# line/open-universe

Measured on AMD Instinct MI355X. Metric: real_time_factor (audio s / wall s), UNIVERSE++ 16 kHz 8-step enhance, higher is better.
Workload: dtype f32; 1 GPU; UNIVERSE++ 16 kHz, 8 diffusion steps, batch=1 utterance(s) of 4 s per GPU per step; network=PP16, n_diffusion_steps=8, batch_per_gpu=1, samples_per_utterance=64000, launches_per_enhance=414

## Files before the change

### open-universe_amd/csrc/ou_api.cpp

```cpp
#include <hip/hip_runtime.h>

#include <cmath>
#include <cstdio>
#include <cstdlib>
#include <cstring>
#include <map>
#include <string>
#include <vector>

#include "../../include/ouniverse.h"
#include "../../include/ouniverse_tuning.h"
#include "ou_kernels.h"
#include "ou_model.h"

using namespace ou;

namespace {
thread_local std::string g_last_error;
constexpr int kMaxSteps = 256;
constexpr size_t kProfSlots = 32768;
constexpr float kInvSqrt2 = 0.70710678118654752440f;
constexpr size_t align256(size_t bytes) { return (bytes + 255) & ~size_t(255); }

struct TensorRef {
  size_t off;
  int C, T;
};
struct Options {
  int dbg = 0, xcd_map = -1, conv_direct = 5, fuse = -1, fuse_nc = 0, rate_small = 1, fuse_upfir = 1, block3 = 0, d4_fir = 1,
      d4_force = 0, d4_short = 1, d2_wk = 0, wino = 1, d2_map = -1, unfuse64 = 0, preact = 1;
  int gru_v = 2, gru_bmax = 0, gru_ts = 0, gru_upw = 0, gru_backoff = 0, gru_agent = -1, gru_dbg = 0;
  int split = -1;
  int dbg_dec0_under_gru = 0;
  int tile_prefetch = 1;
  int trace = 0, no_overlap = 0, ts = 0, deep_factor = 8, mask_fused = 1, split_wino = 1, d2_tile_rule = 1;
  int ens_share = 1;
  double tile_min = -1.0;
  std::string chain_ts;
};
}

struct ou_packer {
  Model m;
  std::map<std::string, HostTensor> sd;
  std::vector<float> blob;
  std::string err;
};

struct ou_handle {
  Model m;
  const float* W = nullptr;
  int device = 0;
  int num_cu = 256;
  std::string err;
  std::map<std::string, TensorRef> tensors;
  int n_launch = 0, n_conv = 0;
  int cond_B = 0, cond_T = 0;
  bool trace = false;
  Options opt;
  std::string plan_with_options;
  int last_cfg = -1;
  long long* tstamps = nullptr;
  std::map<size_t, float> alphas;
  hipStream_t aux[3] = {nullptr, nullptr, nullptr};
  std::vector<hipEvent_t> events;
  size_t ev_used = 0;
  bool overlap = true;
  int force_cfg = -1, force_sc = 0;
  bool profile = false;
  struct ProfRec { double flops, bytes; int cfg; };
  std::vector<ProfRec> prof;
  size_t prof_used = 0;
  unsigned long long* prof_dev = nullptr;
  int fuse_mode = -1;
  int fuse_nc = 0;
  struct WsRec { const void* ws; size_t bytes; int B, T; };
  std::vector<WsRec> ws_ready;
  int gru_agent_stores = 0;
  int lanes = 1, lane = 0;
  int lane_max_b = 0;
  struct NoiseSource {
    bool on = false;
    unsigned long long seed = 0;
    std::vector<unsigned long long> streams;
    float* scratch = nullptr;
    size_t scratch_bytes = 0;
  } noise_src;
  double plane_per_sample = 0.0, wav_plane_per_sample = 0.0;
  bool ws_ok(const void* ws, size_t bytes, int B, int T) const {
    (void)T;
    for (const WsRec& r : ws_ready)
      if (r.ws == ws) return r.B == B && r.bytes <= bytes;
    return false;
  }
};

namespace {

int fail(ou_handle* h, int code, const std::string& msg) {
  if (h) h->err = msg;
  g_last_error = msg;
  return code;
}

struct Tensor {
  float* p = nullptr;
  int C = 0, T = 0;
};

struct OptDesc {
  const char* key;
  int Options::*ip;
  double Options::*dp;
  bool experiments_only;
  const char* doc;
};
const OptDesc kOptions[] = {
    {"conv_direct", &Options::conv_direct, nullptr, false, "kernel generations the conv launcher may use (0 .. 5, ConvArgs::direct)"},
    {"split", &Options::split, nullptr, false, "-1 rule / 0 never / 1 wherever possible: conv_split_kernel (bf16-split operands)"},
    {"split_wino", &Options::split_wino, nullptr, false, "experiments build: 0 = the plain bf16-split kernel also where its minimal-filtering form would take the layer"},
    {"wino", &Options::wino, nullptr, false, "0: never the minimal-filtering (Winograd / Cook-Toom) kernel variants"},
    {"fuse", &Options::fuse, nullptr, false, "-1 cost model / 0 never / 2 / 3: depth of the fused ConvBlock body (conv_chain kernels)"},
    {"fuse_nc", &Options::fuse_nc, nullptr, false, "128 / 256: columns per tile of the fused ConvBlock body (0: launcher's choice)"},
    {"fuse_upfir", &Options::fuse_upfir, nullptr, false, "0: up-path anti-alias FIR always as its own pass"},
    {"rate_small", &Options::rate_small, nullptr, false, "0: outermost rate-change convs on the generic kernels (no rate_down / rate_up)"},
    {"preact", &Options::preact, nullptr, false, "0: every PReLU in its consumer's operand path (ConvArgs::out_act never set)"},
    {"unfuse64", &Options::unfuse64, nullptr, false, "1: 64-channel ConvBlock bodies as three split-K launches"},
    {"block3", &Options::block3, nullptr, false, "1: the three body convs of a deep-level ConvBlock in one launch (experiments build only)"},
    {"xcd_map", &Options::xcd_map, nullptr, false, "block -> tile mapping of the LDS-tiled conv kernel (-1: launcher's choice)"},
    {"d2_map", &Options::d2_map, nullptr, false, "block -> tile mapping of the wide-load split-K kernels (-1: launcher's choice)"},
    {"d2_tile_rule", &Options::d2_tile_rule, nullptr, false, "0: round 5's 64- vs 32-column rule of the wide-load split-K kernels (ignores that only 64-column tiles have minimal filtering)"},
    {"d2_wk", &Options::d2_wk, nullptr, false, "4 / 8: K slices of conv_direct2_kernel (0: launcher's rule)"},
    {"d4_fir", &Options::d4_fir, nullptr, false, "0: up convs with a fusable FIR stay on the first-generation fused kernel"},
    {"d4_short", &Options::d4_short, nullptr, false, "0: the 401-frame levels at batch 1 stay on the first-generation kernels"},
    {"d4_force", &Options::d4_force, nullptr, false, "10 TM + log2(WK): that conv_direct4 tile shape wherever a layer admits it"},
    {"tile_min", nullptr, &Options::tile_min, false, "wave tiles per SIMD from which the no-split-K kernels take a layer (< 0: 1.2)"},
    {"tile_prefetch", &Options::tile_prefetch, nullptr, false, "0: no LDS prefetch of the epilogue operand in conv_direct3_kernel"},
    {"deep_factor", &Options::deep_factor, nullptr, false, "blocks of 64 x 128 per CU up to which a layer counts as 'deep' (split-K kernels)"},
    {"mask_fused", &Options::mask_fused, nullptr, false, "ragged batches: 0 = a separate tail-mask launch after EVERY producer (reference form of the masks)"},
    {"gru_v", &Options::gru_v, nullptr, false, "2 ring kernel / 1 polling-wave kernel (experiments build)"},
    {"gru_bmax", &Options::gru_bmax, nullptr, false, "cap on the utterances per GRU launch (forces the chunked path)"},
    {"gru_upw", &Options::gru_upw, nullptr, false, "hidden units per workgroup of the ring kernel (0: from the batch size)"},
    {"gru_backoff", &Options::gru_backoff, nullptr, false, "poll back-off experiments of the ring kernel (0: none)"},
    {"gru_agent_stores", &Options::gru_agent, nullptr, false, "-1 handle's mode / 0 plain / 1 agent-scope publishes"},
    {"gru_dbg", &Options::gru_dbg, nullptr, false, "bit 0 no republish safety net, bit 1 system-scope publishes, bit 2 FAULT INJECTION (tests)"},
    {"gru_ts", &Options::gru_ts, nullptr, false, "1: per-wave cycle stamps of the GRU kernel into the end of the workspace (tuning)"},
    {"ts", &Options::ts, nullptr, false, "1: per-wave phase stamps in ou_bench_conv (tuning)"},
    {"trace", &Options::trace, nullptr, false, "1: one line per conv launch on stderr"},
    {"no_overlap", &Options::no_overlap, nullptr, false, "1: no side streams inside a call (every kernel alone on the device)"},
    {"ens_share", &Options::ens_share, nullptr, false, "ou_enhance_ensemble: 1 = conditioner once over the B inputs, its results replicated; 0 = over all E * B rows"},
    {"dbg", &Options::dbg, nullptr, true, "phase ablation switches of the conv kernels: WRONG results by design"},
    {"dbg_dec0", &Options::dbg_dec0_under_gru, nullptr, true, "first decoder block under the GRU: upper-bound measurement, WRONG results"},
};
constexpr int kNumOptions = (int)(sizeof(kOptions) / sizeof(kOptions[0]));
const OptDesc* find_option(const char* key) {
  for (int i = 0; i < kNumOptions; i++)
    if (std::strcmp(kOptions[i].key, key) == 0) return &kOptions[i];
  return nullptr;
}
using EnvCfg = Options;

struct Runner {
  ou_handle* h;
  EnvCfg env;
  char* base;
  size_t cap;
  size_t off = 0;
  bool dry;
  hipStream_t st;
  int B;
  hipError_t herr = hipSuccess;
  bool oom = false;
  const char* where = "";
  size_t max_plane = 0;
  bool mel_scale_preset = false;

  Runner(ou_handle* h_, void* ws, size_t cap_, bool dry_, hipStream_t st_, int B_)
      : h(h_), env(h_->opt), base((char*)ws), cap(cap_), dry(dry_), st(st_), B(B_), main_st(st_) {
#ifndef OU_EXPERIMENTS
    env.dbg = 0; env.dbg_dec0_under_gru = 0;
#endif
  }

  float* alloc_raw(size_t floats) {
    size_t bytes = align256(floats * 4);
    size_t o = off;
// ... 67 lines not shown
    const float* res = nullptr;
    float res_scale = 1.f;
    const float* in_scale = nullptr;
    bool act = true;
    const float* fir = nullptr;
    int fir_len = 0;
    const float* fir_bias = nullptr;
    bool rate_down = false;
    bool rate_up = false;
    bool out_act = false;
    float out_alpha = 1.f;
    bool no_mask = false;
  };
  bool stored_act = false;
  bool unsupported = false;
  std::vector<ConvArgs>* collect = nullptr;
  unsigned* status_words = nullptr;
  unsigned long long* block3_bar = nullptr;
  int gru_area_rows = 0;
  bool gru_shared = false;
  hipEvent_t pre_gru = nullptr;
  bool want_pre_gru = false;
  static int gru_share_of(int lanes, int B, bool overlap) {
    const int ncl = 2 * B < 8 ? 2 * B : 8;
    const int by_lanes = lanes > 1 ? (ncl * lanes + 7) / 8 : 1;
    return by_lanes * (overlap ? 2 : 1);
  }

  Tensor conv(const ConvL& L, const Tensor& in, const std::string& name, const Epi& e, const Tensor* dst = nullptr) {
    int Nq, Tout;
    if (L.stride > 1) { Nq = in.T / L.stride; Tout = Nq; }
    else { Nq = in.T; Tout = in.T * L.up; }
    Tensor out = dst ? *dst : alloc(name, L.Cout, Tout);
    if (dry || !ok()) return out;
    ConvArgs a;
    a.x = in.p; a.w = W(L.w_off); a.bias = W(L.b_off); a.y = out.p;
    if (L.KWP) { a.wd = W(L.wd_off); a.wu = W(L.wu_off); }
    if (L.ws_on) a.wsplit = W(L.ws_off);
    if (L.wsw_on) a.wsplitw = W(L.wsw_off);
    a.split = env.split; a.split_wino = env.split_wino;
    a.in_scale = e.in_scale;
    a.act = (L.act && e.act) ? 1 : 0;
    a.alpha_val = a.act ? h->alphas[L.a_off] : 0.f;
    a.add = e.add; a.add_scale = e.add_scale;
    a.film = e.film; a.film_bstride = e.film_bstride;
    a.res = e.res; a.res_scale = e.res_scale;
    if (e.out_act && !collect && !e.fir && !e.rate_down && !e.rate_up) { a.out_act = 1; a.out_alpha = e.out_alpha; }
    stored_act = false;
    if (e.fir && !e.rate_down) { a.fir = e.fir; a.fir_len = e.fir_len; a.bias = e.fir_bias; }
    if (e.rate_down) { a.fir = e.fir; a.fir_len = e.fir ? e.fir_len : 0; }
    a.B = B; a.Cin = L.Cin; a.Tin = in.T; a.Cout = L.Cout; a.M = L.M; a.Mp = L.Mp; a.KW = L.KW;
    a.stride = L.stride; a.pad = L.pad; a.up = L.up; a.CK = L.CK; a.Nq = Nq; a.Tout = Tout;
    a.force_cfg = h->force_cfg; a.force_sc = h->force_sc;
    a.dbg = env.dbg; a.force_xcd_map = env.xcd_map; a.direct = env.conv_direct; a.d4_fir_unfused = env.d4_fir; a.d4_force = env.d4_force; a.d4_short = env.d4_short; a.deep_factor = env.deep_factor; a.d2_tile_rule = env.d2_tile_rule; a.d2_wk = env.d2_wk; a.wino = env.wino; a.d2_map = env.d2_map;
    a.tile_min = env.tile_min; a.tile_prefetch = env.tile_prefetch;
    a.tstamps = h->tstamps;
    if (ragged && env.mask_fused && !e.no_mask) a.lens = lens_of(Tout);
    if (collect) { collect->push_back(a); return out; }
    int cfg = -1;
    if (h->profile && h->prof_dev && h->prof_used < kProfSlots) {
      ou_handle::ProfRec rec;
      const int kref = L.KW;
      rec.flops = 2.0 * L.M * (double)Nq * L.Cin * kref * B;
      rec.bytes = 4.0 * ((double)B * ((double)L.Cin * in.T + (double)L.Cout * Tout) + (double)L.M * L.Cin * kref);
      rec.cfg = -1;
      a.prof = h->prof_dev + 32 * h->prof_used;
      h->prof.push_back(rec);
      h->prof_used++;
    }
    unsupported = false;
    if (e.rate_down) {
      chk(launch_rate_down(a, st, &cfg), L.name.c_str());
    } else if (e.rate_up) {
      chk(launch_rate_up(a, st, &cfg), L.name.c_str());
    } else {
      hipError_t le = launch_conv(a, h->num_cu, st, &cfg);
      if (le == hipErrorNotSupported && a.out_act) {
        a.out_act = 0;
        le = launch_conv(a, h->num_cu, st, &cfg);
      }
      stored_act = a.out_act != 0;
      if (le == hipErrorNotSupported && e.fir) {
        if (a.prof) { h->prof.pop_back(); h->prof_used--; }
        unsupported = true;
        return out;
      }
      chk(le, L.name.c_str());
    }
    if (a.prof) h->prof.back().cfg = cfg;
    h->last_cfg = cfg;
    if (!e.no_mask && !(a.lens && conv_masks_rows(cfg))) mask(out);
    if (h->trace)
      std::fprintf(stderr, "OU_TRACE conv %-64s cfg=%d M=%d Nq=%d K=%d(Cin=%d KW=%d CK=%d) stride=%d up=%d B=%d MFLOP=%.1f\n",
                   name.c_str(), cfg, L.M, Nq, L.Cin * L.KW, L.Cin, L.KW, L.CK, L.stride, L.up, B,
                   2.0 * L.M * Nq * L.Cin * L.KW * B * 1e-6);
    h->n_conv++;
    return out;
  }

  struct BlockOut { Tensor h_next, v, c1; };
  int plan_chain(const BlockL& Bk, int T) {
    h->fuse_mode = env.fuse; h->fuse_nc = env.fuse_nc;
    if (h->fuse_mode == 0) return 0;
    if (ragged && !env.mask_fused) return 0;
    if (h->fuse_mode < 0 && Bk.C % 16 == 0 && Bk.c1.KWP && Bk.c2.KWP && Bk.c3.KWP) {
      if (env.conv_direct >= 3 && direct3_tiles_per_simd(Bk.C, T, B, h->num_cu) >= 1.9 && T >= 1024) return 0;
      if (env.unfuse64 && env.conv_direct >= 5 && env.wino && Bk.C % 64 == 0 && T >= 1024) return 0;
// ... 2335 lines not shown
```

### open-universe_amd/csrc/ou_conv_direct4.hip

```cpp
#include "ou_kernels.h"
#include "ou_internal.h"
#include "ou_dev.h"

#include <cmath>
#include <cstdlib>
#include <type_traits>

namespace ou {

typedef float f32x4acc __attribute__((ext_vector_type(4)));

template <int R, int TM, int WN, int WK, int D>
__global__ __launch_bounds__(64 * WN * WK) void conv_direct4_kernel(ConvArgs p) {
  constexpr int TN = 4, LPS = 2 * R, BM = 16 * TM, NW = WN * WK, EP = 68;
  static_assert(WN == 1 || WK == 1, "a block is either WN column tiles or WK slices of the reduction");
  static_assert(TM >= 1 && TM <= 4, "16 .. 64-row tiles");
  static_assert(D * LPS <= 60, "loads in flight must fit vmcnt");
  static_assert(D == 2 || D == 4, "ring depth");
  typedef float f32x3 __attribute__((ext_vector_type(3)));
  typedef typename std::conditional<TM == 4, f32x4, typename std::conditional<TM == 3, f32x3,
          typename std::conditional<TM == 2, f32x2, float>::type>::type>::type avec;
  extern __shared__ __attribute__((aligned(16))) float smem[];
  const int tid = threadIdx.x, lane = tid & 63;
  const int wv = __builtin_amdgcn_readfirstlane(tid >> 6);
  const int wn = WK == 1 ? wv : 0, wk = WK == 1 ? 0 : wv;
  const int L = blockIdx.x, q8 = L >> 3;
  int rg, cidx;
  if (p.xcd_map == 1) {
    const int gm8 = (p.grid_m + 7) >> 3;
    rg = (q8 % gm8) * 8 + (L & 7);
    cidx = q8 / gm8;
  } else {
    rg = q8 % p.grid_m;
    cidx = (q8 / p.grid_m) * 8 + (L & 7);
  }
  const int b = cidx / p.grid_n, chunk = cidx - b * p.grid_n;
  const int n0 = (chunk * WN + wn) * 64, m0 = rg * BM;
  if (b >= p.B || rg >= p.grid_m) return;
  if (WK == 1 && n0 >= p.Nq) return;
  if (p.prof && tid == 0) atomicMin(p.prof + (blockIdx.x & 15), (unsigned long long)__builtin_amdgcn_s_memrealtime());
  const int l15 = lane & 15, kk = lane >> 4;
  const int Tin = p.Tin, Mp = p.Mp, CK = p.CK, lck = 31 - __clz(CK);
  const float alpha = p.act ? p.alpha_val : 1.0f;
  const u32x4 rx = direct_desc(p.x + (size_t)b * p.Cin * Tin, (unsigned)p.Cin * (unsigned)Tin * 4u);
  const u32x4 rw = direct_desc(p.w, (unsigned)p.Cin * (unsigned)R * (unsigned)Mp * 4u);
  const int avo = (kk * Mp + m0 + TM * l15) * 4;
  const int c0 = n0 + TN * l15;
  const int bvo = c0 < p.Nq ? (kk * Tin + c0 * R) * 4 : (int)0x80000000;

  const int NS = (p.Cin >> 2) / WK;
  avec a4[D][R];
  f32x4 b4[D][R];
#pragma unroll
  for (int d0 = 0; d0 < D; d0++)
#pragma unroll
    for (int k = 0; k < R; k++) {
      if constexpr (TM == 4) a4[d0][k] = f32x4{0.f, 0.f, 0.f, 0.f};
      else if constexpr (TM == 3) a4[d0][k] = f32x3{0.f, 0.f, 0.f};
      else if constexpr (TM == 2) a4[d0][k] = f32x2{0.f, 0.f};
      else a4[d0][k] = 0.f;
      b4[d0][k] = f32x4{0.f, 0.f, 0.f, 0.f};
    }
  f32x4acc acc[TM][TN];
#pragma unroll
  for (int i = 0; i < TM; i++)
#pragma unroll
    for (int j = 0; j < TN; j++) acc[i][j] = f32x4acc{0.f, 0.f, 0.f, 0.f};

#define OU_ISSUE(g_, d)                                                                                                  \
  {                                                                                                                      \
    const int c4 = (wk + WK * (g_)) * 4;                                                                                 \
    const int wrow = ((c4 >> lck) * R) * CK + (c4 & (CK - 1));                   \
    const int xso = c4 * Tin * 4;                                                                                        \
    _Pragma("unroll") for (int k = 0; k < R; k++) {                                                                      \
      if constexpr (TM == 4)                                                                                             \
        asm volatile("buffer_load_dwordx4 %0, %1, %2, %3 offen" : "+v"(a4[d][k]) : "v"(avo), "s"(rw), "s"((wrow + k * CK) * Mp * 4)); \
      else if constexpr (TM == 3)                                                                                        \
        asm volatile("buffer_load_dwordx3 %0, %1, %2, %3 offen" : "+v"(a4[d][k]) : "v"(avo), "s"(rw), "s"((wrow + k * CK) * Mp * 4)); \
      else if constexpr (TM == 2)                                                                                        \
        asm volatile("buffer_load_dwordx2 %0, %1, %2, %3 offen" : "+v"(a4[d][k]) : "v"(avo), "s"(rw), "s"((wrow + k * CK) * Mp * 4)); \
      else                                                                                                               \
        asm volatile("buffer_load_dword %0, %1, %2, %3 offen" : "+v"(a4[d][k]) : "v"(avo), "s"(rw), "s"((wrow + k * CK) * Mp * 4)); \
    }                                                                                                                    \
    _Pragma("unroll") for (int k = 0; k < R; k++)                                                                        \
      asm volatile("buffer_load_dwordx4 %0, %1, %2, %3 offen offset:%4" : "+v"(b4[d][k]) : "v"(bvo), "s"(rx), "s"(xso), "n"(16 * k)); \
  }
#define OU_MMA(d, out)                                                                                                   \
  {                                                                                                                      \
    asm volatile("s_waitcnt vmcnt(%0)" ::"n"((out) * LPS));                                                              \
    _Pragma("unroll") for (int k = 0; k < R; k++) { asm volatile("" : "+v"(a4[d][k])); asm volatile("" : "+v"(b4[d][k])); } \
    float X[4 * R];                                                                                                      \
    _Pragma("unroll") for (int k = 0; k < R; k++) {                                                                      \
// ... 6 lines not shown
        if constexpr (TM == 1) av = a4[d][k]; else av = a4[d][k][i];                                                     \
        _Pragma("unroll") for (int j = 0; j < TN; j++)                                                                   \
          acc[i][j] = __builtin_amdgcn_mfma_f32_16x16x4f32(av, X[j * R + k], acc[i][j], 0, 0, 0);                        \
      }                                                                                                                  \
  }
  const bool ts_on = p.tstamps != nullptr;
  long long tc0 = 0, tc1 = 0, tc2 = 0, tr0 = 0;
  if (ts_on) { tr0 = (long long)__builtin_amdgcn_s_memrealtime(); tc0 = __builtin_readcyclecounter(); }
  if constexpr (D == 4) {
    OU_ISSUE(0, 0); OU_ISSUE(1, 1); OU_ISSUE(2, 2); OU_ISSUE(3, 3);
    if (ts_on) tc1 = __builtin_readcyclecounter();
    const int NR = NS / 4;
    for (int r = 0; r + 1 < NR; r++) {
      const int g = r * 4;
      OU_MMA(0, 3); OU_ISSUE(g + 4, 0);
      OU_MMA(1, 3); OU_ISSUE(g + 5, 1);
      OU_MMA(2, 3); OU_ISSUE(g + 6, 2);
      OU_MMA(3, 3); OU_ISSUE(g + 7, 3);
    }
    OU_MMA(0, 3); OU_MMA(1, 2); OU_MMA(2, 1); OU_MMA(3, 0);
  } else {
    OU_ISSUE(0, 0); OU_ISSUE(1, 1);
    if (ts_on) tc1 = __builtin_readcyclecounter();
    const int NR = NS / 2;
    for (int r = 0; r + 1 < NR; r++) {
      const int g = r * 2;
      OU_MMA(0, 1); OU_ISSUE(g + 2, 0);
      OU_MMA(1, 1); OU_ISSUE(g + 3, 1);
    }
    OU_MMA(0, 1); OU_MMA(1, 0);
  }
  if (ts_on) tc2 = __builtin_readcyclecounter();
#undef OU_ISSUE
#undef OU_MMA

  float* Ew = smem + (size_t)wv * BM * EP;
#pragma unroll
  for (int i = 0; i < TM; i++)
#pragma unroll
    for (int r = 0; r < 4; r++)
      *reinterpret_cast<f32x4*>(&Ew[(TM * (4 * kk + r) + i) * EP + 4 * l15]) =
          f32x4{acc[i][0][r], acc[i][1][r], acc[i][2][r], acc[i][3][r]};
  if constexpr (WK > 1) asm volatile("s_waitcnt lgkmcnt(0)\n\ts_barrier" ::: "memory");
  else asm volatile("s_waitcnt lgkmcnt(0)" ::: "memory");

  const int rt = WK == 1 ? lane : tid;
  constexpr int RNT = WK == 1 ? 64 : 64 * WK;
  const float* Er = WK == 1 ? Ew : smem;
  const float* filmb = p.film ? p.film + (size_t)b * p.film_bstride : nullptr;
  const size_t ybase = (size_t)b * p.Cout * p.Tout;
  const float insc = p.in_scale ? p.in_scale[b] : 1.0f;
  const int nvalid = p.Nq - n0;
  const int rlen = ragged_len(p.lens, b);
  if (p.up == 1) {
    constexpr int NQ = BM * 16, QPT = (NQ + RNT - 1) / RNT;
#pragma unroll
    for (int u = 0; u < QPT; u++) {
      const int e = rt + u * RNT;
      if (NQ % RNT != 0 && e >= NQ) break;
      const int row = e >> 4, cq = (e & 15) * 4;
      const int m = m0 + row;
      if (m >= p.M || cq >= nvalid) continue;
      const size_t idx = ybase + (size_t)m * p.Tout + n0 + cq;
      const bool full = cq + 4 <= nvalid;
      f32x4 ad = {0.f, 0.f, 0.f, 0.f}, rs = {0.f, 0.f, 0.f, 0.f};
      if (full) {
        if (p.add) ad = *reinterpret_cast<const f32x4u*>(p.add + idx);
        if (p.res) rs = *reinterpret_cast<const f32x4u*>(p.res + idx);
      } else {
#pragma unroll
        for (int s = 0; s < 4; s++) {
          if (p.add && cq + s < nvalid) ad[s] = p.add[idx + s];
          if (p.res && cq + s < nvalid) rs[s] = p.res[idx + s];
        }
      }
      f32x4 v = *reinterpret_cast<const f32x4*>(&Er[row * EP + cq]);
#pragma unroll
      for (int k = 1; k < WK; k++) v += *reinterpret_cast<const f32x4*>(&Er[(k * BM + row) * EP + cq]);
      if (p.in_scale) v *= insc;
      v += p.bias[m];
      if (p.add) v = (v + ad) * p.add_scale;
      if (filmb) v = filmb[m] * v + filmb[p.Cout + m];
      if (p.res) v = (v + rs) * p.res_scale;
      if (p.lens) v = ragged_mask4(v, n0 + cq, rlen);
      if (full) {
        *reinterpret_cast<f32x4u*>(p.y + idx) = v;
      } else {
#pragma unroll
        for (int s = 0; s < 4; s++)
          if (cq + s < nvalid) p.y[idx + s] = v[s];
      }
    }
  } else {
    const int up = p.up;
    const int m_hi = (m0 + BM - 1 < p.M - 1) ? m0 + BM - 1 : p.M - 1;
    const int co_lo = (int)__umulhi((unsigned)m0, p.magic_up);
    const int nco = (int)__umulhi((unsigned)m_hi, p.magic_up) - co_lo + 1;
    const int qpc = 16 * up;
    const int total = nco * qpc;
    for (int e = rt; e < total; e += RNT) {
      const int cl = (int)__umulhi((unsigned)(e >> 4), p.magic_up);
      const int tl = (e - cl * qpc) * 4;
      const int co = co_lo + cl;
      const int q0 = (int)__umulhi((unsigned)tl, p.magic_up);
      int ph = tl - q0 * up, q = q0;
      f32x4 v;
      bool ok[4];
// ... 244 lines not shown
    o[0] = tr0; o[1] = tc1 - tc0; o[2] = tc2 - tc1; o[3] = tc3 - tc2; o[4] = tc4 - tc3; o[5] = tc5 - tc4; o[6] = twait;
    o[7] = (long long)__builtin_amdgcn_s_memrealtime();
  }
  if (p.prof && tid == 0) atomicMin(p.prof + 16 + (blockIdx.x & 15), ~(unsigned long long)__builtin_amdgcn_s_memrealtime());
}

struct Direct4wCfg {
  int KW, TM, WK;
  void (*kern)(ConvArgs);
};
#define OU_D4W(KW, TM, WK) {KW, TM, WK, conv_direct4w_kernel<KW, TM, WK>}
static const Direct4wCfg kDirect4wCfgs[] = {OU_D4W(3, 1, 8), OU_D4W(3, 2, 8), OU_D4W(5, 1, 8), OU_D4W(5, 2, 8),
                                            OU_D4W(3, 1, 4), OU_D4W(3, 2, 4), OU_D4W(5, 1, 4), OU_D4W(5, 2, 4)};
hipError_t launch_conv_direct4w(const ConvArgs& a, int num_cu, hipStream_t stream, int* cfg_out) {
  if (!a.wu || a.stride != 1 || a.up != 1 || (a.KW != 3 && a.KW != 5) || a.pad != (a.KW - 1) / 2 || a.fir || a.Cin % 16 ||
      (a.in_scale != nullptr && a.act))
    return hipErrorInvalidConfiguration;
  if ((long)a.Cin * a.Tin * 4 >= (1L << 31) || (long)a.Cin * a.Mp * 8 * 4 >= (1L << 31)) return hipErrorInvalidConfiguration;
  const bool forced = a.force_cfg >= 600 && a.force_cfg < 800;
  if (!forced && !(a.wino && a.direct >= 5)) return hipErrorInvalidConfiguration;
  const int slots = a.Cin / 4;
  const long ct = (a.Nq + 63) / 64;
  int tm = 0, wk = 8;
  if (forced) {
    tm = ((a.force_cfg % 100) / 10);
    wk = a.force_cfg >= 700 ? 4 : 8;
  } else {
    const long b64 = (long)((a.M + 31) / 32) * ct * a.B;
    if (a.Nq >= 1024 || b64 * 10 >= (long)num_cu * 8) return hipErrorInvalidConfiguration;
    long best = 0;
    for (int t = 1; t <= 2; t++) {
      const long blocks = (long)((a.M + 16 * t - 1) / (16 * t)) * ct * a.B;
      const long cost = (blocks + num_cu - 1) / num_cu * t;
      if (!tm || cost <= best) { tm = t; best = cost; }
    }
  }
  if (tm < 1 || tm > 2 || slots % (wk * 4) != 0) return hipErrorInvalidConfiguration;
  const Direct4wCfg* c = nullptr;
  for (const Direct4wCfg& k : kDirect4wCfgs)
    if (k.KW == a.KW && k.TM == tm && k.WK == wk) { c = &k; break; }
  if (!c) return hipErrorInvalidConfiguration;
  ConvArgs aa = a;
  const long gy = (a.M + 16 * tm - 1) / (16 * tm);
  aa.grid_m = (int)gy;
  aa.grid_n = (int)ct;
  const long nblocks = 8L * ((gy + 7) / 8) * ct * a.B;
  if (cfg_out) *cfg_out = (wk == 4 ? 700 : 600) + 10 * tm + a.KW;
  hipLaunchKernelGGL(c->kern, dim3((unsigned)nblocks), dim3(64 * wk), (size_t)wk * 16 * tm * 68 * 4, stream, aa);
  return hipGetLastError();
}

struct Direct4Cfg {
  int R, TM, WN, WK, D;
  void (*kern)(ConvArgs);
};
#define OU_D4(R, TM, WN, WK, D) {R, TM, WN, WK, D, conv_direct4_kernel<R, TM, WN, WK, D>}
#ifdef OU_EXPERIMENTS
#define OU_D4_SHAPES(R, D)                                                                                    \
  OU_D4(R, 4, 4, 1, D), OU_D4(R, 2, 4, 1, D), OU_D4(R, 4, 1, 2, D), OU_D4(R, 2, 1, 2, D), OU_D4(R, 4, 1, 4, D), \
  OU_D4(R, 2, 1, 4, D), OU_D4(R, 4, 1, 8, D), OU_D4(R, 2, 1, 8, D), OU_D4(R, 1, 1, 4, D), OU_D4(R, 1, 1, 8, D), \
  OU_D4(R, 3, 1, 4, D), OU_D4(R, 3, 1, 8, D)
#else
#define OU_D4_SHAPES(R, D)                                                                            \
  OU_D4(R, 2, 4, 1, D), OU_D4(R, 2, 1, 2, D), OU_D4(R, 2, 1, 4, D), OU_D4(R, 2, 1, 8, D), OU_D4(R, 1, 1, 4, D), \
  OU_D4(R, 1, 1, 8, D), OU_D4(R, 3, 1, 4, D), OU_D4(R, 3, 1, 8, D)
#endif
static const Direct4Cfg kDirect4Cfgs[] = {
    OU_D4_SHAPES(1, 4), OU_D4_SHAPES(2, 4), OU_D4_SHAPES(3, 2), OU_D4_SHAPES(4, 2), OU_D4_SHAPES(5, 2), OU_D4_SHAPES(8, 2),
};
static size_t direct4_smem(const Direct4Cfg& c) { return (size_t)c.WN * c.WK * 16 * c.TM * 68 * 4; }
hipError_t init_direct4_kernels() {
  for (const Direct4Cfg& c : kDirect4Cfgs) {
    if (direct4_smem(c) <= 64 * 1024) continue;
    hipError_t e = hipFuncSetAttribute(reinterpret_cast<const void*>(c.kern), hipFuncAttributeMaxDynamicSharedMemorySize,
                                       (int)direct4_smem(c));
    if (e != hipSuccess) return e;
  }
  return hipSuccess;
}

static bool direct4_pick(int M, long ct_b, int slots, int R, int D, bool short_layer, int num_cu, int* tm_out, int* wk_out) {
  if (short_layer) {
    int wk = 8;
    while (wk > 4 && slots % (wk * D) != 0) wk >>= 1;
    if (slots % (wk * D)) return false;
    int best_tm = 0;
    long best_cost = 0;
    for (int tm = 1; tm <= 3; tm++) {
      const long blocks = (long)((M + 16 * tm - 1) / (16 * tm)) * ct_b;
      const long cost = (blocks + num_cu - 1) / num_cu * tm;
      if (!best_tm || cost <= best_cost) { best_tm = tm; best_cost = cost; }
    }
    *tm_out = best_tm; *wk_out = wk;
    return true;
  }
  const long tiles = (long)((M + 31) / 32) * ct_b;
  int wk = 8;
  while (wk > 1 && (slots % (wk * D) != 0 || (slots / wk) * 8 * R < 64 || tiles * wk > 12000)) wk >>= 1;
  if (slots % (wk * D)) return false;
  *tm_out = 2; *wk_out = wk;
  return true;
}

hipError_t launch_conv_direct4(const ConvArgs& a, int num_cu, hipStream_t stream, int* cfg_out, bool probe) {
  const int R = a.stride > 1 ? a.stride : 1;
  if (a.KW != R || a.pad != 0 || (a.stride > 1 && (a.up != 1 || a.Tin != a.Nq * R)) || a.Cin % 16 || a.CK % 4 || a.fir ||
      (a.in_scale != nullptr && a.act))
    return hipErrorInvalidConfiguration;
  if ((long)a.Cin * a.Tin * 4 >= (1L << 31) || (long)a.Cin * a.KW * a.Mp * 4 >= (1L << 31)) return hipErrorInvalidConfiguration;
  if (a.up > 1 && (a.Cout * a.up != a.M || a.Tout != a.Nq * a.up)) return hipErrorInvalidConfiguration;
  const int slots = a.Cin / 4;
  const long ct = (a.Nq + 63) / 64;
  const bool short_layer = a.Nq < 1024 && a.B < 4;
  if (a.force_cfg < 300 && a.d4_force == 0 && short_layer && (!a.d4_short || a.B > 1 || (probe && a.up > 1)))
    return hipErrorInvalidConfiguration;
  const Direct4Cfg* best = nullptr;
  auto code = [](const Direct4Cfg& c) { return 10 * c.TM + (c.WK == 1 ? 0 : c.WK == 2 ? 1 : c.WK == 4 ? 2 : 3); };
  const int D = R <= 2 ? 4 : 2;
  int want = a.force_cfg >= 300 ? a.force_cfg - 300 : a.d4_force;
  for (int pass = 0; pass < 2 && !best; pass++) {
    if (pass == 1) {
      if (a.force_cfg >= 300) break;
      int tm = 0, wk = 0;
      if (!direct4_pick(a.M, ct * a.B, slots, R, D, short_layer, num_cu, &tm, &wk)) break;
      want = 10 * tm + (wk == 1 ? 0 : wk == 2 ? 1 : wk == 4 ? 2 : 3);
    } else if (want == 0) {
      continue;
    }
    for (const Direct4Cfg& c : kDirect4Cfgs)
      if (c.R == R && slots % (c.WK * c.D) == 0 && code(c) == want) { best = &c; break; }
  }
  if (!best) return hipErrorInvalidConfiguration;
  if (a.out_act) return hipErrorNotSupported;
  if (probe) return hipSuccess;
  const Direct4Cfg& c = *best;
  ConvArgs aa = a;
  const long gy = (a.M + 16 * c.TM - 1) / (16 * c.TM);
  aa.grid_m = (int)gy;
  aa.magic_up = a.up == 1 ? 0u : (unsigned)(0x100000000ull / (unsigned)a.up) + 1u;
  const long chunks = (ct + c.WN - 1) / c.WN;
  aa.grid_n = (int)chunks;
  const double xb = (double)a.Cin * a.Tin * a.B, wb = (double)a.M * a.Cin * a.KW;
  aa.xcd_map = wb > xb ? 1 : 2;
  if (a.force_xcd_map == 1 || a.force_xcd_map == 2) aa.xcd_map = a.force_xcd_map;
  const long nblocks = aa.xcd_map == 1 ? 8L * ((gy + 7) / 8) * chunks * a.B : (chunks * a.B + 7) / 8 * 8 * gy;
  if (cfg_out) *cfg_out = 300 + code(c);
  hipLaunchKernelGGL(c.kern, dim3((unsigned)nblocks), dim3(64 * c.WN * c.WK), direct4_smem(c), stream, aa);
  return hipGetLastError();
}

}
```

### open-universe_amd/csrc/ou_conv_mfma.hip

```cpp
#include "ou_kernels.h"
#include "ou_internal.h"
#include "ou_dev.h"

#include <cmath>
#include <cstdlib>
#include <type_traits>

namespace ou {

constexpr int CONV_XCAP = 4096;
constexpr int CONV_XCAP_BIG = 8192;

template <int TM, int TN, int WM, int WN, int WK, int CONV_MAXW, int U, bool EXACT>
__global__ __launch_bounds__(64 * WM * WN * WK) void conv_mfma_kernel(ConvArgs p) {
  constexpr int CONV_NT = 64 * WM * WN * WK;
  constexpr int XCAP = (WK == 8 && TM * TN == 4) ? CONV_XCAP_BIG : CONV_XCAP;
  constexpr int CONV_MAXX = XCAP / CONV_NT;
  static_assert(WM * WN * WK == 4 || WM * WN * WK == 8, "4 or 8 waves per block");
  constexpr int BM = 32 * TM * WM, BN = 32 * TN * WN;
  extern __shared__ __attribute__((aligned(16))) float smem[];

  const int tid = threadIdx.x, lane = tid & 63;
  const int wave = __builtin_amdgcn_readfirstlane(tid >> 6);
  const int kw = wave % WK, wn = (wave / WK) % WN, wm = wave / (WK * WN);
// ... 362 lines not shown
    OU_CONV_CFG_OFF(64, 64, 8, 12, 512),
#endif
};
constexpr int kNumConvCfgs = sizeof(kConvCfgs) / sizeof(kConvCfgs[0]);

static size_t conv_smem_bytes(const ConvCfg& c, const ConvArgs& a) {
  int span = (c.BN - 1) * a.stride + a.KW;
  size_t xt_al = ((size_t)a.SC * a.CK * span + 3) & ~size_t(3);
  size_t stage = 2 * (xt_al + (size_t)a.SC * a.CK * a.KW * c.BM) + 2 * c.BM;
  if (c.WK == 8) stage += 2 * 4 * c.WK;
  size_t epi = (size_t)c.WK * c.BM * (c.BN + 4);
  return 4 * (stage > epi ? stage : epi);
}

hipError_t init_conv_kernels() {
  hipError_t e_d3 = hipSuccess;
  for (int i = 0; i < kNumConvCfgs; i++) {
    if (!kConvCfgs[i].kern4) continue;
    hipError_t e = hipFuncSetAttribute(reinterpret_cast<const void*>(kConvCfgs[i].kern4),
                                       hipFuncAttributeMaxDynamicSharedMemorySize, 160 * 1024);
    if (e != hipSuccess) return e;
    e = hipFuncSetAttribute(reinterpret_cast<const void*>(kConvCfgs[i].kern2),
                            hipFuncAttributeMaxDynamicSharedMemorySize, 160 * 1024);
    if (e != hipSuccess) return e;
    e = hipFuncSetAttribute(reinterpret_cast<const void*>(kConvCfgs[i].kern_g),
                            hipFuncAttributeMaxDynamicSharedMemorySize, 160 * 1024);
    if (e != hipSuccess) return e;
  }
  e_d3 = init_direct3_kernels();
  if (e_d3 != hipSuccess) return e_d3;
  e_d3 = init_block3_kernels();
  if (e_d3 != hipSuccess) return e_d3;
  e_d3 = init_direct4_kernels();
  if (e_d3 != hipSuccess) return e_d3;
  e_d3 = init_split_kernels();
  if (e_d3 != hipSuccess) return e_d3;
  return init_chain_kernels();
}

bool conv_masks_rows(int cfg) { return cfg >= 0 && !(cfg >= 100 && cfg < 200); }

namespace {
hipError_t try_split(const ConvArgs& a, int num_cu, hipStream_t stream, int* cfg_out) {
  if (!a.wsplit || a.split == 0) return hipErrorInvalidConfiguration;
  const double tiles = (double)(a.M / 64) * ((a.Nq + 127) / 128) * a.B / 4.0;
  const bool rule = a.M >= 256 && a.M % 256 == 0 && tiles >= ((a.Nq < 1024 || a.KW == 5) ? 0.45 : 0.9) * num_cu;
  if (!(a.split == 1 || a.force_cfg >= 800 || rule)) return hipErrorInvalidConfiguration;
  return launch_conv_split(a, num_cu, stream, cfg_out);
}
hipError_t try_direct3(const ConvArgs& a, int num_cu, hipStream_t stream, int* cfg_out) {
  if (a.direct < 3) return hipErrorInvalidConfiguration;
  return launch_conv_direct3(a, num_cu, stream, cfg_out);
}
hipError_t try_direct4(const ConvArgs& a, int num_cu, hipStream_t stream, int* cfg_out) {
  if (a.direct < 4) return hipErrorInvalidConfiguration;
  if (a.fir) {
    if (a.d4_fir_unfused && a.force_cfg < 0) {
      ConvArgs probe = a;
      probe.fir = nullptr; probe.fir_len = 0;
      if (launch_conv_direct4(probe, num_cu, stream, nullptr, true) == hipSuccess) return hipErrorNotSupported;
    }
    return a.force_cfg >= 0 ? hipErrorNotSupported : hipErrorInvalidConfiguration;
  }
  return launch_conv_direct4(a, num_cu, stream, cfg_out, false);
}
hipError_t try_direct4w(const ConvArgs& a, int num_cu, hipStream_t stream, int* cfg_out) {
  if (a.direct < 5) return hipErrorInvalidConfiguration;
  return launch_conv_direct4w(a, num_cu, stream, cfg_out);
}
hipError_t try_direct(const ConvArgs& a, int num_cu, hipStream_t stream, int* cfg_out) {
  if (a.direct == 0) return hipErrorInvalidConfiguration;
  const long wide = (long)((a.M + 63) / 64) * ((a.Nq + 127) / 128) * a.B;
  const bool wide_ok = a.wd && a.direct >= 2 && a.stride == 1 && a.up == 1;
  const bool deep = ((a.Nq <= 16384 || wide_ok) && wide < (long)a.deep_factor * num_cu) || a.force_cfg >= 100;
  if (!deep) return hipErrorInvalidConfiguration;
  return launch_conv_direct(a, num_cu, stream, cfg_out);
}
struct ConvFamily {
  int lo, hi;
  bool final_if_forced;
  hipError_t (*attempt)(const ConvArgs&, int, hipStream_t, int*);
};
const ConvFamily kConvFamilies[] = {
    {800, 1100, true, try_split},
    {200, 300, true, try_direct3},
    {300, 500, true, try_direct4},
    {600, 800, true, try_direct4w},
    {100, 200, false, try_direct},
};
bool forced_into(const ConvFamily& f, int cfg) {
  if (cfg >= f.lo && cfg < f.hi) return true;
  return f.attempt == try_direct3 && cfg >= 500 && cfg < 600;
}
}

hipError_t launch_conv(const ConvArgs& a, int num_cu, hipStream_t stream, int* cfg_out) {
  if (a.Cin % a.CK || a.CK < 2 || (a.CK & (a.CK - 1)) || a.Mp % 64 || a.Nq <= 0) return hipErrorInvalidValue;
  for (const ConvFamily& f : kConvFamilies) {
    const bool forced = a.force_cfg >= 0 && forced_into(f, a.force_cfg);
    if (a.force_cfg >= 0 && !forced) continue;
    const hipError_t e = f.attempt(a, num_cu, stream, cfg_out);
    if (e != hipErrorInvalidConfiguration) return e;
    if (forced && f.final_if_forced) return e;
  }
  if (a.fir) return hipErrorNotSupported;
  int pick = -1;
  for (int i = 0; i < kNumConvCfgs; i++) {
    const ConvCfg& c = kConvCfgs[i];
    if (a.force_cfg >= 0 && i != a.force_cfg) continue;
    if (!c.kern4) continue;
// ... 64 lines not shown
```

### open-universe_amd/csrc/ou_kernels.h

```cpp
#pragma once
#include <hip/hip_runtime.h>

#include <cstddef>
#include <cstdint>

namespace ou {

struct ConvArgs {
  const float* x = nullptr;
  const float* w = nullptr;
  const float* wd = nullptr;
  const float* wu = nullptr;
  const void* wsplit = nullptr;
  const void* wsplitw = nullptr;
  int split_wino = 1;
  const float* bias = nullptr;
  float* y = nullptr;
  const float* in_scale = nullptr;
  int act = 0;
  float alpha_val = 0.f;
  const float* add = nullptr;
  const float* film = nullptr;
  const float* res = nullptr;
  float add_scale = 1.f, res_scale = 1.f;
  int film_bstride = 0;
  int B = 1, Cin = 0, Tin = 0, Cout = 0, M = 0, Mp = 0, KW = 1, stride = 1, pad = 0, up = 1, CK = 2;
  int Nq = 0;
  int Tout = 0;
  unsigned magic_span[3] = {0, 0, 0};
  unsigned magic_up = 0;
  int SC = 1;
  int grid_n = 1, grid_m = 1;
  int xcd_map = 0;
  int force_cfg = -1, force_sc = 0;
  int force_xcd_map = -1;
  double tile_min = -1.0;
  int tile_prefetch = 1;
  int direct = 5;
  int d2_map = -1;
  int split = -1;
  int wino = 1;
  int d2_wk = 0;
  int d4_fir_unfused = 1;
  int d4_short = 1;
  int d4_force = 0;
  int d2_tile_rule = 1;
  int deep_factor = 8;
  int out_act = 0;
  float out_alpha = 1.f;
  const int* lens = nullptr;
  const float* fir = nullptr;
  int fir_len = 0;
  int tile_bm = 32, tile_bn = 0, tile_halo = 0;
  int dbg = 0;
  long long* tstamps = nullptr;
  unsigned long long* prof = nullptr;
};
hipError_t launch_conv(const ConvArgs& a, int num_cu, hipStream_t stream, int* cfg_out = nullptr);
bool conv_masks_rows(int cfg);
hipError_t init_conv_kernels();
double direct3_tiles_per_simd(int M, int Nq, int B, int num_cu);
bool rate_down_supported(const ConvArgs& a);
hipError_t launch_rate_down(const ConvArgs& a, hipStream_t st, int* cfg_out = nullptr);
bool rate_up_supported(const ConvArgs& a);
hipError_t launch_rate_up(const ConvArgs& a, hipStream_t st, int* cfg_out = nullptr);

struct StepCoef {
  float w_in, sigma_net, w_skip, w_out, sig2, c1, s_next, beta;
};
enum OutMode { OUT_SCORE = 0, OUT_UPDATE = 1 };
hipError_t launch_in_conv(const float* x, const float* w, const float* bias, const StepCoef* coef, int coef_bstride,
                          float* y, int B, int C, int T, int KW, hipStream_t s, const int* lens = nullptr);
hipError_t launch_out_conv(const float* s, const float* w, const float* bias, const float* alphas, const float* x,
                           const float* noise, float* out, const StepCoef* coef, int coef_bstride, int edm,
                           int mode, int B, int C, int T, int KW, hipStream_t st, const int* lens = nullptr);

hipError_t launch_sigma_embed(const StepCoef* coef, int S, const float* params, int simple, int n_rff, int D,
                              float* g, hipStream_t st);
hipError_t launch_film(const float* g, const float* W, const float* b, float* film, int S, int rows, int D,
                       hipStream_t st);
struct CoefBlock { StepCoef c[64]; };
hipError_t launch_upload_coef(StepCoef* dst, const CoefBlock& blk, int n, hipStream_t st);

struct RowInfo { int t_raw, pad_left, t_pad, _r; };
constexpr int kMaxLenLevels = 8;
struct LevelSpec { int n = 0; int num[kMaxLenLevels]; int den[kMaxLenLevels]; };
struct RowBlock { int t_raw[64]; };
hipError_t launch_upload_rows(RowInfo* rows, int* lens, const RowBlock& blk, int n, int off, int B, int tot_ds,
                              const LevelSpec& lv, hipStream_t st);
hipError_t launch_mask_tail(float* y, const int* lens, int B, int C, int T, hipStream_t st);
hipError_t launch_gru_tail_fill(float* gx, const int* lens, int B, int H, int T, hipStream_t st);
hipError_t launch_pad_normalize_var(const float* mix, float* y, float* stats, const RowInfo* rows, int B, int T_raw_max,
                                    int T_pad_max, float level, hipStream_t st);
hipError_t launch_post_var(const float* x, const float* stats, float* out, const RowInfo* rows, int B, int T_raw_max,
                           int T_pad_max, int keep_rms, int peak_guard, hipStream_t st);

// ... 174 lines not shown
```

Baseline: 604.0 x_realtime.

## Fuse up-path anti-alias FIR into conv_direct4 epilogue with overlapping tiles

Adds a FIR-fused variant of conv_direct4_kernel for transposed/up convs. The upsampled outputs are reduced in LDS, and the anti-alias FIR plus bias and residual are applied in the epilogue. Column tiles of 62 frames overlap by one frame on each side to provide the FIR halo, and row tiles are rounded to multiples of the up factor. It becomes the default (d4_fir=2), replacing a separate FIR pass after conv_direct4 and removing one launch plus an intermediate round trip. The trade-offs are redundant halo computation and more register/LDS pressure in the epilogue.

```diff
diff --git a/open-universe_amd/csrc/ou_api.cpp b/open-universe_amd/csrc/ou_api.cpp
--- a/open-universe_amd/csrc/ou_api.cpp
+++ b/open-universe_amd/csrc/ou_api.cpp
@@ -27,7 +27,7 @@
   int C, T;
 };
 struct Options {
-  int dbg = 0, xcd_map = -1, conv_direct = 5, fuse = -1, fuse_nc = 0, rate_small = 1, fuse_upfir = 1, block3 = 0, d4_fir = 1,
+  int dbg = 0, xcd_map = -1, conv_direct = 5, fuse = -1, fuse_nc = 0, rate_small = 1, fuse_upfir = 1, block3 = 0, d4_fir = 2,
       d4_force = 0, d4_short = 1, d2_wk = 0, wino = 1, d2_map = -1, unfuse64 = 0, preact = 1;
   int gru_v = 2, gru_bmax = 0, gru_ts = 0, gru_upw = 0, gru_backoff = 0, gru_agent = -1, gru_dbg = 0;
   int split = -1;
@@ -131,7 +131,7 @@
     {"d2_map", &Options::d2_map, nullptr, false, "block -> tile mapping of the wide-load split-K kernels (-1: launcher's choice)"},
     {"d2_tile_rule", &Options::d2_tile_rule, nullptr, false, "0: round 5's 64- vs 32-column rule of the wide-load split-K kernels (ignores that only 64-column tiles have minimal filtering)"},
     {"d2_wk", &Options::d2_wk, nullptr, false, "4 / 8: K slices of conv_direct2_kernel (0: launcher's rule)"},
-    {"d4_fir", &Options::d4_fir, nullptr, false, "0: up convs with a fusable FIR stay on the first-generation fused kernel"},
+    {"d4_fir", &Options::d4_fir, nullptr, false, "up convs with a fusable FIR: 2 = FIR in conv_direct4_kernel's epilogue, 1 = conv_direct4_kernel + FIR pass, 0 = first-generation fused kernel"},
     {"d4_short", &Options::d4_short, nullptr, false, "0: the 401-frame levels at batch 1 stay on the first-generation kernels"},
     {"d4_force", &Options::d4_force, nullptr, false, "10 TM + log2(WK): that conv_direct4 tile shape wherever a layer admits it"},
     {"tile_min", nullptr, &Options::tile_min, false, "wave tiles per SIMD from which the no-split-K kernels take a layer (< 0: 1.2)"},
@@ -305,7 +305,7 @@
     a.B = B; a.Cin = L.Cin; a.Tin = in.T; a.Cout = L.Cout; a.M = L.M; a.Mp = L.Mp; a.KW = L.KW;
     a.stride = L.stride; a.pad = L.pad; a.up = L.up; a.CK = L.CK; a.Nq = Nq; a.Tout = Tout;
     a.force_cfg = h->force_cfg; a.force_sc = h->force_sc;
-    a.dbg = env.dbg; a.force_xcd_map = env.xcd_map; a.direct = env.conv_direct; a.d4_fir_unfused = env.d4_fir; a.d4_force = env.d4_force; a.d4_short = env.d4_short; a.deep_factor = env.deep_factor; a.d2_tile_rule = env.d2_tile_rule; a.d2_wk = env.d2_wk; a.wino = env.wino; a.d2_map = env.d2_map;
+    a.dbg = env.dbg; a.force_xcd_map = env.xcd_map; a.direct = env.conv_direct; a.d4_fir = env.d4_fir; a.d4_force = env.d4_force; a.d4_short = env.d4_short; a.deep_factor = env.deep_factor; a.d2_tile_rule = env.d2_tile_rule; a.d2_wk = env.d2_wk; a.wino = env.wino; a.d2_map = env.d2_map;
     a.tile_min = env.tile_min; a.tile_prefetch = env.tile_prefetch;
     a.tstamps = h->tstamps;
     if (ragged && env.mask_fused && !e.no_mask) a.lens = lens_of(Tout);
diff --git a/open-universe_amd/csrc/ou_conv_direct4.hip b/open-universe_amd/csrc/ou_conv_direct4.hip
--- a/open-universe_amd/csrc/ou_conv_direct4.hip
+++ b/open-universe_amd/csrc/ou_conv_direct4.hip
@@ -10,7 +10,110 @@
 
 typedef float f32x4acc __attribute__((ext_vector_type(4)));
 
-template <int R, int TM, int WN, int WK, int D>
+template <int UP, int BM, int WK>
+__device__ __forceinline__ void d4_fir_up(const ConvArgs& p, float* E, int rt, int b, int m0, int n0) {
+  constexpr int EP = 68, RNT = WK == 1 ? 64 : 64 * WK, MB = (BM / UP) * UP, NCO = BM / UP, NTAP = 2 * UP + 1, WIN = NTAP + 3;
+  constexpr int NQ = BM * 16, QPT = (NQ + RNT - 1) / RNT;
+  constexpr int QPC = 16 * UP, TOTAL = NCO * QPC, NIT = (TOTAL + RNT - 1) / RNT;
+  constexpr bool PRE = NIT <= 2;
+  const int rlen = ragged_len(p.lens, b);
+  const size_t ybase = (size_t)b * p.Cout * p.Tout;
+  const int co0 = m0 / UP;
+  const int lo = n0 > 0 ? UP : 0;
+  auto quad = [&](int e, int& cl, int& tl, size_t& idx, bool (&ok)[4]) {
+    cl = e / QPC;
+    tl = (e - cl * QPC) * 4;
+    const int co = co0 + cl;
+    const long t = (long)n0 * UP + tl;
+    idx = ybase + (size_t)co * p.Tout + (size_t)t;
+#pragma unroll
+    for (int s = 0; s < 4; s++) ok[s] = e < TOTAL && co < p.Cout && tl + s >= lo && tl + s < 63 * UP && t + s < p.Tout;
+  };
+  f32x4 rs_pre[PRE ? NIT : 1];
+  if constexpr (PRE) {
+#pragma unroll
+    for (int k = 0; k < NIT; k++) {
+      int cl, tl; size_t idx; bool ok[4];
+      quad(rt + k * RNT, cl, tl, idx, ok);
+      f32x4 rs = {0.f, 0.f, 0.f, 0.f};
+      if (p.res) {
+        if (ok[0] && ok[1] && ok[2] && ok[3]) rs = *reinterpret_cast<const f32x4u*>(p.res + idx);
+        else {
+#pragma unroll
+          for (int s = 0; s < 4; s++) if (ok[s]) rs[s] = p.res[idx + s];
+        }
+      }
+      rs_pre[k] = rs;
+    }
+  }
+#pragma unroll
+  for (int u = 0; u < QPT; u++) {
+    const int e = rt + u * RNT;
+    if (NQ % RNT != 0 && e >= NQ) break;
+    const int row = e >> 4, cq = (e & 15) * 4;
+    f32x4 v = *reinterpret_cast<const f32x4*>(&E[row * EP + cq]);
+#pragma unroll
+    for (int k = 1; k < WK; k++) v += *reinterpret_cast<const f32x4*>(&E[(k * BM + row) * EP + cq]);
+    const int ph = row % UP;
+    const bool rowok = row < MB && m0 + row < p.M;
+#pragma unroll
+    for (int s = 0; s < 4; s++) {
+      const int fr = n0 + cq + s;
+      if (!rowok || fr >= p.Nq || fr * UP + ph >= rlen) v[s] = 0.f;
+    }
+    *reinterpret_cast<f32x4*>(&E[row * EP + cq]) = v;
+  }
+  if constexpr (WK > 1) asm volatile("s_waitcnt lgkmcnt(0)\n\ts_barrier" ::: "memory");
+  else asm volatile("s_waitcnt lgkmcnt(0)" ::: "memory");
+  float f[NTAP];
+#pragma unroll
+  for (int j = 0; j < NTAP; j++) f[j] = p.fir[j];
+#pragma unroll
+  for (int k = 0; k < NIT; k++) {
+    const int e = rt + k * RNT;
+    int cl, tl; size_t idx; bool ok[4];
+    quad(e, cl, tl, idx, ok);
+    if (!(ok[0] || ok[1] || ok[2] || ok[3])) continue;
+    const bool full = ok[0] && ok[1] && ok[2] && ok[3];
+    f32x4 rs = {0.f, 0.f, 0.f, 0.f};
+    if constexpr (PRE) rs = rs_pre[k];
+    else if (p.res) {
+      if (full) rs = *reinterpret_cast<const f32x4u*>(p.res + idx);
+      else {
+#pragma unroll
+        for (int s = 0; s < 4; s++) if (ok[s]) rs[s] = p.res[idx + s];
+      }
+    }
+    const float* zrow = E + (cl * UP) * EP;
+    int fq = tl / UP - 1, ph = tl % UP;
+    float win[WIN];
+#pragma unroll
+    for (int i = 0; i < WIN; i++) {
+      const float z = zrow[ph * EP + (fq < 0 ? 0 : fq)];
+      win[i] = fq < 0 ? 0.f : z;
+      if (++ph == UP) { ph = 0; fq++; }
+    }
+    const float bb = p.bias[co0 + cl];
+    f32x4 o;
+#pragma unroll
+    for (int s = 0; s < 4; s++) {
+      float acc = 0.f;
+#pragma unroll
+      for (int j = 0; j < NTAP; j++) acc = fmaf(f[j], win[s + j], acc);
+      acc += bb;
+      if (p.res) acc = (acc + rs[s]) * p.res_scale;
+      o[s] = acc;
+    }
+    if (p.lens) o = ragged_mask4(o, n0 * UP + tl, rlen);
+    if (full) *reinterpret_cast<f32x4u*>(p.y + idx) = o;
+    else {
+#pragma unroll
+      for (int s = 0; s < 4; s++) if (ok[s]) p.y[idx + s] = o[s];
+    }
+  }
+}
+
+template <int R, int TM, int WN, int WK, int D, bool FIR = false>
 __global__ __launch_bounds__(64 * WN * WK) void conv_direct4_kernel(ConvArgs p) {
   constexpr int TN = 4, LPS = 2 * R, BM = 16 * TM, NW = WN * WK, EP = 68;
   static_assert(WN == 1 || WK == 1, "a block is either WN column tiles or WK slices of the reduction");
@@ -35,9 +138,9 @@
     cidx = (q8 / p.grid_m) * 8 + (L & 7);
   }
   const int b = cidx / p.grid_n, chunk = cidx - b * p.grid_n;
-  const int n0 = (chunk * WN + wn) * 64, m0 = rg * BM;
+  const int n0 = (chunk * WN + wn) * (FIR ? 62 : 64), m0 = rg * (FIR ? p.tile_bm : BM);
   if (b >= p.B || rg >= p.grid_m) return;
-  if (WK == 1 && n0 >= p.Nq) return;
+  if (WK == 1 && (FIR && n0 > 0 ? n0 + 1 : n0) >= p.Nq) return;
   if (p.prof && tid == 0) atomicMin(p.prof + (blockIdx.x & 15), (unsigned long long)__builtin_amdgcn_s_memrealtime());
   const int l15 = lane & 15, kk = lane >> 4;
   const int Tin = p.Tin, Mp = p.Mp, CK = p.CK, lck = 31 - __clz(CK);
@@ -150,7 +253,16 @@
   const float insc = p.in_scale ? p.in_scale[b] : 1.0f;
   const int nvalid = p.Nq - n0;
   const int rlen = ragged_len(p.lens, b);
-  if (p.up == 1) {
+  if constexpr (FIR) {
+    float* Ef = WK == 1 ? Ew : smem;
+    switch (p.up) {
+      case 2: d4_fir_up<2, BM, WK>(p, Ef, rt, b, m0, n0); break;
+      case 3: d4_fir_up<3, BM, WK>(p, Ef, rt, b, m0, n0); break;
+      case 4: d4_fir_up<4, BM, WK>(p, Ef, rt, b, m0, n0); break;
+      case 5: d4_fir_up<5, BM, WK>(p, Ef, rt, b, m0, n0); break;
+      default: d4_fir_up<8, BM, WK>(p, Ef, rt, b, m0, n0); break;
+    }
+  } else if (p.up == 1) {
     constexpr int NQ = BM * 16, QPT = (NQ + RNT - 1) / RNT;
 #pragma unroll
     for (int u = 0; u < QPT; u++) {
@@ -501,9 +613,11 @@
 
 struct Direct4Cfg {
   int R, TM, WN, WK, D;
+  bool fir;
   void (*kern)(ConvArgs);
 };
-#define OU_D4(R, TM, WN, WK, D) {R, TM, WN, WK, D, conv_direct4_kernel<R, TM, WN, WK, D>}
+#define OU_D4(R, TM, WN, WK, D) {R, TM, WN, WK, D, false, conv_direct4_kernel<R, TM, WN, WK, D>}
+#define OU_D4F(TM, WN, WK) {1, TM, WN, WK, 4, true, conv_direct4_kernel<1, TM, WN, WK, 4, true>}
 #ifdef OU_EXPERIMENTS
 #define OU_D4_SHAPES(R, D)                                                                                    \
   OU_D4(R, 4, 4, 1, D), OU_D4(R, 2, 4, 1, D), OU_D4(R, 4, 1, 2, D), OU_D4(R, 2, 1, 2, D), OU_D4(R, 4, 1, 4, D), \
@@ -516,6 +630,8 @@
 #endif
 static const Direct4Cfg kDirect4Cfgs[] = {
     OU_D4_SHAPES(1, 4), OU_D4_SHAPES(2, 4), OU_D4_SHAPES(3, 2), OU_D4_SHAPES(4, 2), OU_D4_SHAPES(5, 2), OU_D4_SHAPES(8, 2),
+    OU_D4F(2, 4, 1), OU_D4F(2, 1, 2), OU_D4F(2, 1, 4), OU_D4F(2, 1, 8), OU_D4F(1, 1, 4), OU_D4F(1, 1, 8), OU_D4F(3, 1, 4),
+    OU_D4F(3, 1, 8),
 };
 static size_t direct4_smem(const Direct4Cfg& c) { return (size_t)c.WN * c.WK * 16 * c.TM * 68 * 4; }
 hipError_t init_direct4_kernels() {
@@ -528,7 +644,9 @@
   return hipSuccess;
 }
 
-static bool direct4_pick(int M, long ct_b, int slots, int R, int D, bool short_layer, int num_cu, int* tm_out, int* wk_out) {
+static int d4_fir_rows(int tm, int fir_up) { return fir_up ? (16 * tm / fir_up) * fir_up : 16 * tm; }
+static bool direct4_pick(int M, long ct_b, int slots, int R, int D, bool short_layer, int num_cu, int fir_up, int* tm_out,
+                         int* wk_out) {
   if (short_layer) {
     int wk = 8;
     while (wk > 4 && slots % (wk * D) != 0) wk >>= 1;
@@ -536,7 +654,8 @@
     int best_tm = 0;
     long best_cost = 0;
     for (int tm = 1; tm <= 3; tm++) {
-      const long blocks = (long)((M + 16 * tm - 1) / (16 * tm)) * ct_b;
+      const int rows = d4_fir_rows(tm, fir_up);
+      const long blocks = (long)((M + rows - 1) / rows) * ct_b;
       const long cost = (blocks + num_cu - 1) / num_cu * tm;
       if (!best_tm || cost <= best_cost) { best_tm = tm; best_cost = cost; }
     }
@@ -553,39 +672,46 @@
 
 hipError_t launch_conv_direct4(const ConvArgs& a, int num_cu, hipStream_t stream, int* cfg_out, bool probe) {
   const int R = a.stride > 1 ? a.stride : 1;
-  if (a.KW != R || a.pad != 0 || (a.stride > 1 && (a.up != 1 || a.Tin != a.Nq * R)) || a.Cin % 16 || a.CK % 4 || a.fir ||
+  const bool fir = a.fir != nullptr;
+  if (a.KW != R || a.pad != 0 || (a.stride > 1 && (a.up != 1 || a.Tin != a.Nq * R)) || a.Cin % 16 || a.CK % 4 ||
       (a.in_scale != nullptr && a.act))
+    return hipErrorInvalidConfiguration;
+  if (fir && ((a.up != 2 && a.up != 3 && a.up != 4 && a.up != 5 && a.up != 8) || R != 1 || a.fir_len != 2 * a.up + 1 || a.add ||
+              a.film || a.in_scale || a.out_act))
     return hipErrorInvalidConfiguration;
   if ((long)a.Cin * a.Tin * 4 >= (1L << 31) || (long)a.Cin * a.KW * a.Mp * 4 >= (1L << 31)) return hipErrorInvalidConfiguration;
   if (a.up > 1 && (a.Cout * a.up != a.M || a.Tout != a.Nq * a.up)) return hipErrorInvalidConfiguration;
   const int slots = a.Cin / 4;
-  const long ct = (a.Nq + 63) / 64;
+  const long ct = fir ? (a.Nq > 63 ? (a.Nq - 1 + 61) / 62 : 1) : (a.Nq + 63) / 64;
   const bool short_layer = a.Nq < 1024 && a.B < 4;
   if (a.force_cfg < 300 && a.d4_force == 0 && short_layer && (!a.d4_short || a.B > 1 || (probe && a.up > 1)))
     return hipErrorInvalidConfiguration;
   const Direct4Cfg* best = nullptr;
   auto code = [](const Direct4Cfg& c) { return 10 * c.TM + (c.WK == 1 ? 0 : c.WK == 2 ? 1 : c.WK == 4 ? 2 : 3); };
   const int D = R <= 2 ? 4 : 2;
-  int want = a.force_cfg >= 300 ? a.force_cfg - 300 : a.d4_force;
+  int want = a.force_cfg >= 350 ? a.force_cfg - 350 : a.force_cfg >= 300 ? a.force_cfg - 300 : a.d4_force;
+  if (a.force_cfg >= 300 && (a.force_cfg >= 350) != fir) return hipErrorInvalidConfiguration;
   for (int pass = 0; pass < 2 && !best; pass++) {
     if (pass == 1) {
       if (a.force_cfg >= 300) break;
       int tm = 0, wk = 0;
-      if (!direct4_pick(a.M, ct * a.B, slots, R, D, short_layer, num_cu, &tm, &wk)) break;
+      if (!direct4_pick(a.M, ct * a.B, slots, R, D, short_layer, num_cu, fir ? a.up : 0, &tm, &wk)) break;
       want = 10 * tm + (wk == 1 ? 0 : wk == 2 ? 1 : wk == 4 ? 2 : 3);
     } else if (want == 0) {
       continue;
     }
     for (const Direct4Cfg& c : kDirect4Cfgs)
-      if (c.R == R && slots % (c.WK * c.D) == 0 && code(c) == want) { best = &c; break; }
+      if (c.R == R && c.fir == fir && slots % (c.WK * c.D) == 0 && code(c) == want) { best = &c; break; }
   }
   if (!best) return hipErrorInvalidConfiguration;
   if (a.out_act) return hipErrorNotSupported;
   if (probe) return hipSuccess;
   const Direct4Cfg& c = *best;
   ConvArgs aa = a;
-  const long gy = (a.M + 16 * c.TM - 1) / (16 * c.TM);
+  const int rows = d4_fir_rows(c.TM, fir ? a.up : 0);
+  const long gy = (a.M + rows - 1) / rows;
   aa.grid_m = (int)gy;
+  aa.tile_bm = rows;
   aa.magic_up = a.up == 1 ? 0u : (unsigned)(0x100000000ull / (unsigned)a.up) + 1u;
   const long chunks = (ct + c.WN - 1) / c.WN;
   aa.grid_n = (int)chunks;
@@ -593,7 +719,7 @@
   aa.xcd_map = wb > xb ? 1 : 2;
   if (a.force_xcd_map == 1 || a.force_xcd_map == 2) aa.xcd_map = a.force_xcd_map;
   const long nblocks = aa.xcd_map == 1 ? 8L * ((gy + 7) / 8) * chunks * a.B : (chunks * a.B + 7) / 8 * 8 * gy;
-  if (cfg_out) *cfg_out = 300 + code(c);
+  if (cfg_out) *cfg_out = (fir ? 350 : 300) + code(c);
   hipLaunchKernelGGL(c.kern, dim3((unsigned)nblocks), dim3(64 * c.WN * c.WK), direct4_smem(c), stream, aa);
   return hipGetLastError();
 }
diff --git a/open-universe_amd/csrc/ou_conv_mfma.hip b/open-universe_amd/csrc/ou_conv_mfma.hip
--- a/open-universe_amd/csrc/ou_conv_mfma.hip
+++ b/open-universe_amd/csrc/ou_conv_mfma.hip
@@ -438,10 +438,19 @@
   if (a.direct < 3) return hipErrorInvalidConfiguration;
   return launch_conv_direct3(a, num_cu, stream, cfg_out);
 }
+bool direct4_fir_rule(const ConvArgs& a) {
+  (void)a;
+  return true;
+}
 hipError_t try_direct4(const ConvArgs& a, int num_cu, hipStream_t stream, int* cfg_out) {
   if (a.direct < 4) return hipErrorInvalidConfiguration;
   if (a.fir) {
-    if (a.d4_fir_unfused && a.force_cfg < 0) {
+    const bool forced = a.force_cfg >= 350 && a.force_cfg < 400;
+    if (forced || (a.d4_fir == 2 && a.force_cfg < 0 && direct4_fir_rule(a))) {
+      const hipError_t e = launch_conv_direct4(a, num_cu, stream, cfg_out, false);
+      if (e != hipErrorInvalidConfiguration || forced) return e == hipErrorInvalidConfiguration ? hipErrorNotSupported : e;
+    }
+    if (a.d4_fir != 0 && a.force_cfg < 0) {
       ConvArgs probe = a;
       probe.fir = nullptr; probe.fir_len = 0;
       if (launch_conv_direct4(probe, num_cu, stream, nullptr, true) == hipSuccess) return hipErrorNotSupported;
diff --git a/open-universe_amd/csrc/ou_kernels.h b/open-universe_amd/csrc/ou_kernels.h
--- a/open-universe_amd/csrc/ou_kernels.h
+++ b/open-universe_amd/csrc/ou_kernels.h
@@ -41,7 +41,7 @@
   int split = -1;
   int wino = 1;
   int d2_wk = 0;
-  int d4_fir_unfused = 1;
+  int d4_fir = 2;
   int d4_short = 1;
   int d4_force = 0;
   int d2_tile_rule = 1;
```

New measurement: 610.3 x_realtime (median of 6 runs). About the same (+1.0%).
